# adria0/plonk-by-fingers

Measured on AMD Instinct MI355X. Metric: NTT elements/sec (Goldilocks, n=2^20 per GPU, natural order, bit-exact vs src/fft.rs), higher is better.
Workload: dtype u64 (Goldilocks p=2^64-2^32+1); 1 GPU; Goldilocks forward NTT, batch 32 x 2^20; n_per_gpu=1048576, n_global=1048576, batch=32, passes=default (2^20: 10,10)

## Files before the change

plonk-by-fingers_amd/csrc/ntt_gl.hpp:

```cpp
#pragma once
#include "ntt_kernels.hpp"

#ifdef PBF_GL_NOMATH
#define PBF_GL_MATH(x) do { } while (0)
#else
#define PBF_GL_MATH(x) x
#endif
#ifdef PBF_GL_NOMEM
#define PBF_GL_NOMEM_ON 1
#else
#define PBF_GL_NOMEM_ON 0
#endif

namespace pbf {

struct GlPassArgs {
  const uint64_t* in;
  uint64_t* out;
  const uint64_t* twpass;
  const uint64_t* tw0;
  const uint64_t* tw1;
  const uint64_t* tc;
  const uint64_t* tws_a;
  const uint64_t* tws_b;
  uint64_t n;
  uint32_t log_n;
  uint32_t log_ns;
  uint32_t tw_bits;
  uint32_t blocks_per_poly;
  uint32_t batch;
  uint32_t scaled;
  uint32_t out_split_log;
  uint32_t xcd_kmajor;
  uint64_t in_pitch, out_pitch;
  const uint64_t* post_tw;
  uint32_t skip_pass_tw;
  const uint64_t* cs_tab;
  const uint64_t* cs_tab1;
  uint32_t cs_bits;
  uint64_t cs_len;
};

template <int K>
__device__ __forceinline__ uint64_t gl_pow2(uint64_t x) {
  constexpr int RAW = ((K % 192) + 192) % 192;
  if constexpr (RAW == 0) {
    return x;
  } else if constexpr (RAW > 160) {
    return gl_div_pow2<192 - RAW>(x);
  } else {
    using T = ShiftKind<RAW>;
    const uint64_t y = apply_shift<Goldilocks, T>(x);
    if constexpr (T::NEG) {
      const FieldArgs f{};
      return Goldilocks::sub(0, y, f);
    } else {
      return y;
    }
  }
}

template <int E64, int Q1, int S2 = 1>
__device__ __forceinline__ void gl_stage_b_twiddle(uint64_t* v) {
  if constexpr (S2 < 16) {
    v[S2] = gl_pow2<(E64 * S2 * Q1) % 192>(v[S2]);
    gl_stage_b_twiddle<E64, Q1, S2 + 1>(v);
  }
}

template <int E64, int Q, int E = 1>
__device__ __forceinline__ void gl_post_twiddle_br(uint64_t* v) {
  if constexpr (E < 16) {
    v[bitrev_c(E, 4)] = gl_pow2<(E64 * E * Q) % 192>(v[bitrev_c(E, 4)]);
    gl_post_twiddle_br<E64, Q, E + 1>(v);
  }
}
template <int E64, int WV, int U = 0>
__device__ __forceinline__ void gl_rg3_c_shift(uint64_t* x) {
  if constexpr (U < 4) {
    constexpr int g = WV + 4 * U;
    x[U * 4 + 1] = gl_pow2<(E64 * g) % 192>(x[U * 4 + 1]);
    x[U * 4 + 2] = gl_pow2<(E64 * 2 * g) % 192>(x[U * 4 + 2]);
    x[U * 4 + 3] = gl_pow2<(E64 * 3 * g) % 192>(x[U * 4 + 3]);
    gl_rg3_c_shift<E64, WV, U + 1>(x);
  }
}

template <int LOGR, int TILE>
struct GlShape {
  static constexpr int R = 1 << LOGR;
  static constexpr int LOGC = LOGR - 6;
  static constexpr int C = 1 << LOGC;
  static constexpr int W = TILE / R;
  static constexpr int NT = TILE / 16;
  static constexpr int WPQ = NT / 256;
#ifdef PBF_GL_PAD_Y
  static constexpr bool YX = false;
#else
  static constexpr bool YX = W == 16 && C > 1;
#endif
  static constexpr int YP = (YX ? 64 : 65) * W;
  static constexpr int LDS = (C * YP > TILE) ? C * YP : TILE;
  static constexpr bool LDS32K = LDS * 8 <= 32768;
  static constexpr int NSUB_C = (64 * W) / NT;
  __host__ __device__ static constexpr int ysw(int k1) {
    return W <= 32 ? (k1 / (32 / W)) & (W - 1) : (k1 & 31);
  }
  __host__ __device__ static constexpr int yidx(int r2, int k1, int w) {
    return r2 * YP + (YX ? (k1 ^ (r2 & 1)) : k1) * W + (w ^ ysw(k1));
  }
};

__device__ __forceinline__ void gl_tile_coords(const GlPassArgs& a, uint32_t tile, uint32_t tiles, uint32_t* poly,
                                               uint32_t* kb) {
  if (a.xcd_kmajor == 1) {
    const uint32_t v = (tile & 7) * (tiles >> 3) + (tile >> 3);
    *kb = v / a.batch;
    *poly = v % a.batch;
  } else if (a.xcd_kmajor == 2) {
    const uint32_t v = (tile & 7) * (tiles >> 3) + (tile >> 3);
    *poly = v / a.blocks_per_poly;
    *kb = v % a.blocks_per_poly;
  } else {
    *poly = tile / a.blocks_per_poly;
    *kb = tile % a.blocks_per_poly;
  }
}

__device__ __forceinline__ uint64_t gl_cs_factor(const GlPassArgs& a, uint64_t i) {
  const FieldArgs f{};
  if (a.cs_tab1) return Goldilocks::mul(a.cs_tab[i & ((1ull << a.cs_bits) - 1)], a.cs_tab1[i >> a.cs_bits], f);
  return a.cs_tab[i];
}

constexpr int GL_STORES = 16;

template <int LOGR, int E64, bool FIRST, int TILE, int RG = 0, int CS = 0>
__device__ __forceinline__ void gl_tile(const GlPassArgs& a, uint64_t* lds, uint32_t tile, uint32_t tiles, int t) {
  using Sh = GlShape<LOGR, TILE>;
  constexpr int C = Sh::C, LOGC = Sh::LOGC, W = Sh::W, NT = Sh::NT, YP = Sh::YP;
  (void)YP;
  static_assert(Sh::NSUB_C * C == GL_STORES, "stores per thread");
  static_assert(RG == 0 || (LOGR == 8 && TILE == 4096 && FIRST == (RG == 1)), "RG shape");
  static_assert(CS == 0 || (FIRST == (CS == 1) && (RG == 0 || RG == 2 * CS - 1)), "CS 1: first pass, CS 2: last pass");
  const FieldArgs f{};
  using G = Goldilocks;
  uint32_t poly, kb;
  gl_tile_coords(a, tile, tiles, &poly, &kb);
  if constexpr (PBF_GL_NOMEM_ON) kb &= 1, poly = 0;
  const uint64_t j0 = (uint64_t)kb * W;
  const uint64_t* in = a.in + (uint64_t)poly * a.in_pitch;
  const uint64_t stride = a.n >> LOGR;

  uint64_t v[16];
  if constexpr (CS == 1) {
#pragma unroll
    for (int h = 0; h < 2; ++h) {
      uint64_t tw[8];
#pragma unroll
      for (int uu = 0; uu < 2; ++uu) {
        const int idx = t + NT * (2 * h + uu);
        const int w = idx % W, r2 = (idx / W) % C, s2 = idx / (C * W);
#pragma unroll
        for (int s1 = 0; s1 < 4; ++s1) {
          const uint64_t i = (j0 + w) + (uint64_t)(16 * C * s1 + C * s2 + r2) * stride;
          const bool on = i < a.cs_len;
          v[8 * h + uu * 4 + s1] = on ? in[i] : 0;
          tw[uu * 4 + s1] = on ? gl_cs_factor(a, i) : 0;
        }
      }
#pragma unroll
      for (int m = 0; m < 8; ++m) v[8 * h + m] = G::mul(v[8 * h + m], tw[m], f);
    }
  } else {
#pragma unroll
    for (int u = 0; u < 4; ++u) {
      const int idx = t + NT * u;
      const int w = idx % W, r2 = (idx / W) % C, s2 = idx / (C * W);
#pragma unroll
      for (int s1 = 0; s1 < 4; ++s1) {
        const int r = 16 * C * s1 + C * s2 + r2;
        v[u * 4 + s1] = in[(j0 + w) + (uint64_t)r * stride];
      }
    }
  }
  uint64_t t3[RG == 3 ? 2 : 1];
  if constexpr (RG == 3) {
    const int wave = t >> 6, q1 = wave / Sh::WPQ, rw = (wave % Sh::WPQ) * 64 + (t & 63);
    const int r2 = rw / W, w = rw % W;
    const uint64_t X = ((uint64_t)q1 << 16) + j0 + w;
    t3[0] = a.tws_a[((uint64_t)r2 << 18) + X];
    t3[1] = a.tws_b[X];
  }
  if constexpr (!FIRST && RG != 3) if (!a.skip_pass_tw) {
    const uint64_t kmask = (1ull << a.log_ns) - 1;
#pragma unroll
    for (int h = 0; h < 2; ++h) {
      uint64_t tw[8];
#pragma unroll
      for (int uu = 0; uu < 2; ++uu) {
        const int u = 2 * h + uu;
        const int idx = t + NT * u;
        const int w = idx % W, r2 = (idx / W) % C, s2 = idx / (C * W);
        const uint64_t k = (j0 + w) & kmask;
#pragma unroll
        for (int s1 = 0; s1 < 4; ++s1) {
          const uint64_t r = (uint64_t)(16 * C * s1 + C * s2 + r2);
          if (a.twpass) {
            tw[uu * 4 + s1] = a.twpass[(r << a.log_ns) + k];
          } else if (a.tws_a) {
            tw[uu * 4 + s1] = G::mul(a.tws_b[(uint64_t)kb * Sh::R + r], a.tws_a[r * W + w], f);
          } else {
            const uint64_t e = ((r * k) << (a.log_n - a.log_ns - LOGR)) & (a.n - 1);
            tw[uu * 4 + s1] = G::mul(a.tw0[e & ((1ull << a.tw_bits) - 1)], a.tw1[e >> a.tw_bits], f);
          }
        }
      }
#pragma unroll
      for (int m = 0; m < 8; ++m) PBF_GL_MATH(v[8 * h + m] = G::mul(v[8 * h + m], tw[m], f));
#ifdef PBF_GL_NOMATH
#pragma unroll
      for (int m = 0; m < 8; ++m) v[8 * h + m] ^= tw[m];
#endif
    }
  }
#pragma unroll
  for (int u = 0; u < 4; ++u) PBF_GL_MATH((dft_reg<G, 2, sub_root_exp(E64, 2)>(v + u * 4, nullptr, f)));
#pragma unroll
  for (int u = 0; u < 4; ++u) {
    const int idx = t + NT * u;
    const int s2 = idx / (C * W), rw = idx % (C * W);
#pragma unroll
    for (int q1 = 0; q1 < 4; ++q1) lds[(q1 * 16 + s2) * (C * W) + rw] = v[u * 4 + bitrev_c(q1, 2)];
  }
  __syncthreads();

  {
    const int wave = t >> 6;
    const int q1 = wave / Sh::WPQ;
    const int rw = (wave % Sh::WPQ) * 64 + (t & 63);
#pragma unroll
    for (int s2 = 0; s2 < 16; ++s2) v[s2] = lds[(q1 * 16 + s2) * (C * W) + rw];
#ifndef PBF_GL_NOMATH
    if constexpr (RG == 3) {
      uint64_t p = t3[0];
      const uint64_t d = t3[1];
#pragma unroll
      for (int s2 = 0; s2 < 16; ++s2) {
        v[s2] = G::mul(v[s2], p, f);
        if (s2 < 15) p = G::mul(p, d, f);
      }
    } else {
      switch (__builtin_amdgcn_readfirstlane(q1)) {
        case 1: gl_stage_b_twiddle<E64, 1>(v); break;
        case 2: gl_stage_b_twiddle<E64, 2>(v); break;
        case 3: gl_stage_b_twiddle<E64, 3>(v); break;
        default: break;
      }
    }
    dft_reg<G, 4, sub_root_exp(E64, 4)>(v, nullptr, f);
#endif
    __syncthreads();
    const int r2 = rw / W, w = rw % W;
#pragma unroll
    for (int q2 = 0; q2 < 16; ++q2) {
      const int k1 = q1 + 4 * q2;
      lds[Sh::yidx(r2, k1, w)] = v[bitrev_c(q2, 4)];
    }
  }
  __syncthreads();

  auto c_map = [&](int u, int* k1, int* w) {
    const int idx = t + NT * u;
    if constexpr (FIRST) {
      *k1 = idx & 63;
      *w = idx >> 6;
    } else {
      *k1 = idx / W;
      *w = idx % W;
    }
  };
  uint64_t x[Sh::NSUB_C * C];
#pragma unroll
  for (int u = 0; u < Sh::NSUB_C; ++u) {
    int k1, w;
    c_map(u, &k1, &w);
#pragma unroll
    for (int r2 = 0; r2 < C; ++r2) x[u * C + r2] = lds[Sh::yidx(r2, k1, w)];
  }
  if constexpr (RG == 3) {
    switch (__builtin_amdgcn_readfirstlane(t >> 6)) {
      case 0: gl_rg3_c_shift<E64, 0>(x); break;
      case 1: gl_rg3_c_shift<E64, 1>(x); break;
      case 2: gl_rg3_c_shift<E64, 2>(x); break;
      default: gl_rg3_c_shift<E64, 3>(x); break;
    }
  } else if constexpr (RG == 1) {
    const uint64_t* tc = a.tc + ((j0 >> 12) & 15) * 256;
#pragma unroll
    for (int u = 0; u < Sh::NSUB_C; ++u) {
      int k1, w;
      c_map(u, &k1, &w);
      uint64_t tw[C];
#pragma unroll
      for (int r2 = 0; r2 < C; ++r2) tw[r2] = tc[r2 * 64 + k1];
#pragma unroll
      for (int r2 = 0; r2 < C; ++r2) x[u * C + r2] = G::mul(x[u * C + r2], tw[r2], f);
    }
  } else {
    uint64_t tw[Sh::NSUB_C * C];
    const int r2lo = a.scaled ? 0 : 1;
#pragma unroll
    for (int u = 0; u < Sh::NSUB_C; ++u) {
      int k1, w;
      c_map(u, &k1, &w);
#pragma unroll
      for (int r2 = 0; r2 < C; ++r2) tw[u * C + r2] = (r2 >= r2lo) ? a.tc[r2 * 64 + k1] : 1;
    }
    if (a.scaled) {
#pragma unroll
      for (int m = 0; m < Sh::NSUB_C * C; ++m) PBF_GL_MATH(x[m] = G::mul(x[m], tw[m], f));
    } else {
#pragma unroll
      for (int u = 0; u < Sh::NSUB_C; ++u)
#pragma unroll
        for (int r2 = 1; r2 < C; ++r2) {
          PBF_GL_MATH(x[u * C + r2] = G::mul(x[u * C + r2], tw[u * C + r2], f));
#ifdef PBF_GL_NOMATH
          x[u * C + r2] ^= tw[u * C + r2];
#endif
        }
    }
  }
  if constexpr (C > 1) {
#pragma unroll
    for (int u = 0; u < Sh::NSUB_C; ++u) PBF_GL_MATH((dft_reg<G, LOGC, sub_root_exp(E64, LOGC)>(x + u * C, nullptr, f)));
  }

  if constexpr (FIRST) {
    uint64_t* o = a.out + (uint64_t)poly * a.out_pitch;
#pragma unroll
    for (int u = 0; u < Sh::NSUB_C; ++u) {
      int k1, w;
      c_map(u, &k1, &w);
      const uint64_t base = (j0 + w) << LOGR;
      if (a.post_tw) {
        uint64_t tw[C];
#pragma unroll
        for (int k2 = 0; k2 < C; ++k2) tw[k2] = a.post_tw[base + k1 + 64 * k2];
#pragma unroll
        for (int k2 = 0; k2 < C; ++k2) x[u * C + bitrev_c(k2, LOGC)] = G::mul(x[u * C + bitrev_c(k2, LOGC)], tw[k2], f);
      }
#pragma unroll
      for (int k2 = 0; k2 < C; ++k2)
        if (!PBF_GL_NOMEM_ON || x[u * C + bitrev_c(k2, LOGC)] == 0x123456789ull)
          o[base + k1 + 64 * k2] = x[u * C + bitrev_c(k2, LOGC)];
    }
  } else {
    const uint64_t ns_mask = (1ull << a.log_ns) - 1;
    uint64_t* out = a.out + (uint64_t)poly * a.out_pitch;
    const uint32_t sl = a.out_split_log;
#pragma unroll
    for (int u = 0; u < Sh::NSUB_C; ++u) {
      int k1, w;
      c_map(u, &k1, &w);
      const uint64_t j = j0 + w;
      const uint64_t base = ((j >> a.log_ns) << (a.log_ns + LOGR)) + (j & ns_mask);
      if (sl == 0) {
        if constexpr (CS == 2) {
          uint64_t tw[C];
#pragma unroll
          for (int k2 = 0; k2 < C; ++k2) tw[k2] = gl_cs_factor(a, base + ((uint64_t)(k1 + 64 * k2) << a.log_ns));
#pragma unroll
          for (int k2 = 0; k2 < C; ++k2) x[u * C + bitrev_c(k2, LOGC)] = G::mul(x[u * C + bitrev_c(k2, LOGC)], tw[k2], f);
        }
#pragma unroll
        for (int k2 = 0; k2 < C; ++k2)
          if (!PBF_GL_NOMEM_ON || x[u * C + bitrev_c(k2, LOGC)] == 0x123456789ull)
            out[base + ((uint64_t)(k1 + 64 * k2) << a.log_ns)] = x[u * C + bitrev_c(k2, LOGC)];
      } else {
        const uint64_t smask = (1ull << sl) - 1;
#pragma unroll
        for (int k2 = 0; k2 < C; ++k2) {
          const uint64_t kk = base + ((uint64_t)(k1 + 64 * k2) << a.log_ns);
          a.out[((((kk >> sl) * a.batch) + poly) << sl) + (kk & smask)] = x[u * C + bitrev_c(k2, LOGC)];
        }
      }
    }
  }
}

template <int LOGR, int TILE>
__device__ __forceinline__ void gl_shape_checks() {
  using Sh = GlShape<LOGR, TILE>;
  static_assert(LOGR >= 6 && LOGR <= 10, "radix 2^6 .. 2^10");
  static_assert(Sh::LDS * 8 <= (TILE > 8192 ? 160 : 80) * 1024, "LDS budget");
  static_assert(Sh::W >= 8 && Sh::WPQ >= 1, "tile shape");
}

template <int LOGR, int E64, bool FIRST, int TILE, int RG = 0, int CS = 0>
__global__ void __launch_bounds__(TILE / 16)
__attribute__((amdgpu_waves_per_eu((FIRST || RG) && GlShape<LOGR, TILE>::LDS32K ? 5 : 4)))
ntt_gl_pass_kernel(GlPassArgs a) {
  gl_shape_checks<LOGR, TILE>();
  __shared__ __attribute__((aligned(16))) uint64_t lds[GlShape<LOGR, TILE>::LDS];
  const uint32_t tiles = a.blocks_per_poly * a.batch;
  gl_tile<LOGR, E64, FIRST, TILE, RG, CS>(a, lds, blockIdx.x, tiles, threadIdx.x);
}

template <int E64>
__global__ void __launch_bounds__(256) __attribute__((amdgpu_waves_per_eu(4))) ntt_gl_rg2_kernel(GlPassArgs a) {
  constexpr int W = 16;
  __shared__ __attribute__((aligned(16))) uint64_t lds[16 * 16 * W];
  const FieldArgs f{};
  using G = Goldilocks;
  const uint32_t tiles = a.blocks_per_poly * a.batch;
  uint32_t poly, kb;
  gl_tile_coords(a, blockIdx.x, tiles, &poly, &kb);
  const int t = threadIdx.x, w = t % W, a1h = t / W;
  const uint64_t j0 = (uint64_t)kb * W, j = j0 + w;
  const uint32_t c = (uint32_t)(j0 >> 6) & 3, a1l = (uint32_t)(j0 >> 14) & 3;
  const uint64_t* in = a.in + (uint64_t)poly * a.in_pitch;
  const uint64_t stride = a.n >> 8;
  uint64_t v[16], tw[16];
#pragma unroll
  for (int a2l = 0; a2l < 16; ++a2l) v[a2l] = in[j + (uint64_t)(a2l * 16 + a1h) * stride];
  const uint64_t* t2 = a.twpass + ((uint64_t)(a1l + 4 * a1h) << 12) + (j & 255);
#pragma unroll
  for (int d = 0; d < 16; ++d) tw[d] = t2[256 * d];
  switch (__builtin_amdgcn_readfirstlane(c)) {
    case 1: gl_stage_b_twiddle<E64, 1>(v); break;
    case 2: gl_stage_b_twiddle<E64, 2>(v); break;
    case 3: gl_stage_b_twiddle<E64, 3>(v); break;
    default: break;
  }
  dft_reg<G, 4, sub_root_exp(E64, 4)>(v, nullptr, f);
#pragma unroll
  for (int d = 0; d < 16; ++d) lds[d * 256 + (a1h ^ (d & 3)) * W + w] = G::mul(v[bitrev_c(d, 4)], tw[d], f);
  __syncthreads();
  const int d2 = t / W;
#pragma unroll
  for (int h = 0; h < 16; ++h) v[h] = lds[d2 * 256 + (h ^ (d2 & 3)) * W + w];
  dft_reg<G, 4, sub_root_exp(E64, 4)>(v, nullptr, f);
  switch (__builtin_amdgcn_readfirstlane(a1l)) {
    case 1: gl_post_twiddle_br<E64, 1>(v); break;
    case 2: gl_post_twiddle_br<E64, 2>(v); break;
    case 3: gl_post_twiddle_br<E64, 3>(v); break;
    default: break;
  }
  uint64_t* out = a.out + (uint64_t)poly * a.out_pitch;
  const uint64_t base = ((j >> 8) << 16) + (j & 255);
#pragma unroll
  for (int e = 0; e < 16; ++e) out[base + ((uint64_t)(d2 + 16 * e) << 8)] = v[bitrev_c(e, 4)];
}

}
```

plonk-by-fingers_amd/csrc/ntt_kernels.hpp:

```cpp
#pragma once
#include "field.hpp"

namespace pbf {

#ifdef PBF_NTT_TIMING_MODES
#define PBF_DBG(a, bit) (((a).dbg & (bit)) != 0)
#else
#define PBF_DBG(a, bit) false
#endif

struct PassArgs {
  const uint64_t* in;
  uint64_t* out;
  const uint64_t* tw0;
  const uint64_t* tw1;
  const uint64_t* rtab;
  const uint64_t* twfull;
  const uint64_t* twpass;
  uint64_t n;
  uint64_t n_inv;
  uint32_t log_n;
  uint32_t log_ns;
  uint32_t tw_bits;
  uint32_t blocks_per_poly;
// ... 5 lines not shown
  uint32_t xcd_kmajor;
  FieldArgs f;
};

__host__ __device__ constexpr int ntt_nstages(int logr, int lq) { return (logr + lq - 1) / lq; }
__host__ __device__ constexpr int ntt_stage_logq(int logr, int s, int lq) {
  return (logr % lq == 0) ? lq : (s == 0 ? logr % lq : lq);
}
__host__ __device__ constexpr int ntt_stage_logl(int logr, int s, int lq) {
  int l = 0;
  for (int i = 0; i < s; ++i) l += ntt_stage_logq(logr, i, lq);
  return l;
}
__host__ __device__ constexpr int bitrev_c(int x, int bits) {
  int r = 0;
  for (int i = 0; i < bits; ++i) r |= ((x >> i) & 1) << (bits - 1 - i);
  return r;
}

template <class F>
__device__ __forceinline__ uint64_t tw_pow(const PassArgs& a, uint64_t e) {
  uint64_t lo = a.tw0[e & ((1ull << a.tw_bits) - 1)];
  uint64_t hi = a.tw1[e >> a.tw_bits];
  return F::mul(lo, hi, a.f);
}

template <int RAW_>
struct ShiftKind {
  static constexpr int RAW = ((RAW_ % 192) + 192) % 192;
  static constexpr bool NEG0 = RAW >= 96;
  static constexpr int S0 = NEG0 ? RAW - 96 : RAW;
  static constexpr bool DIV = S0 > 64;
  static constexpr bool NEG = DIV ? !NEG0 : NEG0;
  static constexpr int S = DIV ? 96 - S0 : S0;
};
template <int E, int LOGQ, int H, int A>
struct TwShift : ShiftKind<(E * A * ((1 << LOGQ) / (2 * H))) % 192> {};

template <class F, class T>
__device__ __forceinline__ uint64_t apply_shift(uint64_t d) {
  if constexpr (T::DIV) return gl_div_pow2<T::S>(d);
  else return F::template mul_pow2<T::S>(d);
}

template <class F, int LOGQ, int E, int H, int A>
__device__ __forceinline__ void dif_bfly(uint64_t* v, int blk, const uint64_t* wq, const FieldArgs& f) {
  constexpr int Q = 1 << LOGQ;
  const uint64_t x = v[blk + A], y = v[blk + A + H];
  v[blk + A] = F::add(x, y, f);
  if constexpr (A == 0) {
    v[blk + A + H] = F::sub(x, y, f);
  } else if constexpr (E < 0) {
    v[blk + A + H] = F::mul(F::sub(x, y, f), wq[A * (Q / (2 * H))], f);
  } else {
    using T = TwShift<E, LOGQ, H, A>;
    const uint64_t d = T::NEG ? F::sub(y, x, f) : F::sub(x, y, f);
    v[blk + A + H] = apply_shift<F, T>(d);
  }
}

template <class F, int LOGQ, int E, int H, int A>
__device__ __forceinline__ void dif_row(uint64_t* v, const uint64_t* wq, const FieldArgs& f) {
  if constexpr (A < H) {
    constexpr int Q = 1 << LOGQ;
#pragma unroll
    for (int blk = 0; blk < Q; blk += 2 * H) dif_bfly<F, LOGQ, E, H, A>(v, blk, wq, f);
    dif_row<F, LOGQ, E, H, A + 1>(v, wq, f);
  }
}

template <class F, int LOGQ, int E, int H>
__device__ __forceinline__ void dif_levels(uint64_t* v, const uint64_t* wq, const FieldArgs& f) {
  if constexpr (H >= 1) {
    dif_row<F, LOGQ, E, H, 0>(v, wq, f);
    dif_levels<F, LOGQ, E, H / 2>(v, wq, f);
  }
}

template <class F, int LOGQ, int E>
__device__ __forceinline__ void dft_reg(uint64_t* v, const uint64_t* wq, const FieldArgs& f) {
  dif_levels<F, LOGQ, E, (1 << LOGQ) / 2>(v, wq, f);
}

__host__ __device__ constexpr int sub_root_exp(int e64, int logq) {
  return e64 < 0 ? -1 : (e64 * (64 >> logq)) % 192;
}

template <bool DB>
__device__ __forceinline__ void tile_barrier() {
  if constexpr (DB) {
    asm volatile("s_waitcnt lgkmcnt(0)" ::: "memory");
    __builtin_amdgcn_s_barrier();
  } else {
    __syncthreads();
  }
}

template <int LOGR, int W, int NT, int LQ>
__device__ __forceinline__ void tile_load(uint64_t* v, const PassArgs& a, const uint64_t* in, uint64_t j0, int t) {
  constexpr int R = 1 << LOGR;
  constexpr int PER = (R * W) / NT;
  constexpr int Q = 1 << ntt_stage_logq(LOGR, 0, LQ);
#pragma unroll
  for (int u = 0; u < PER / Q; ++u) {
    const int sub = t + NT * u;
    const int w = sub % W, i = sub / W;
#pragma unroll
    for (int c = 0; c < Q; ++c) {
      const int r = i + c * (R / Q);
      v[u * Q + c] = PBF_DBG(a, 1) ? (uint64_t)(t * 0x9E3779B9u + r) * 0x100000001ull
                                 : in[(j0 + w) + (uint64_t)r * (a.n >> LOGR)];
    }
  }
}

template <class F, int LOGR, int W, int NT, int LQ, int E64, int S>
__device__ __forceinline__ void ntt_stage(uint64_t* v, uint64_t* buf, const uint64_t* rt, const uint64_t* wq,
                                          const PassArgs& a, uint64_t* out, uint64_t j0, int t) {
  constexpr int R = 1 << LOGR;
  constexpr int PER = (R * W) / NT;
  constexpr int NST = ntt_nstages(LOGR, LQ);
  constexpr int LOGQ = ntt_stage_logq(LOGR, S, LQ);
  constexpr int Q = 1 << LOGQ;
  constexpr int L = 1 << ntt_stage_logl(LOGR, S, LQ);
  constexpr int NSUB = PER / Q;
  constexpr bool LAST = (S == NST - 1);
  const uint64_t n = a.n;
  if constexpr (S == 0) {
    if (a.log_ns > 0) {
      const uint64_t kmask = (1ull << a.log_ns) - 1;
      if (a.twpass) {
        uint64_t tw[PER];
#pragma unroll
        for (int u = 0; u < NSUB; ++u) {
          const int sub = t + NT * u;
          const int w = sub % W, i = sub / W;
          const uint64_t k = (j0 + w) & kmask;
#pragma unroll
          for (int c = 0; c < Q; ++c) tw[u * Q + c] = a.twpass[((uint64_t)(i + c * (R / Q)) << a.log_ns) + k];
        }
#pragma unroll
        for (int m = 0; m < PER; ++m) v[m] = F::mul(v[m], tw[m], a.f);
      } else {
#pragma unroll
        for (int u = 0; u < NSUB; ++u) {
          const int sub = t + NT * u;
          const int w = sub % W, i = sub / W;
          const uint64_t k = (j0 + w) & kmask;
#pragma unroll
          for (int c = 0; c < Q; ++c) {
            const uint64_t r = i + c * (R / Q);
            const uint64_t e = ((r * k) << (a.log_n - a.log_ns - LOGR)) & (n - 1);
            if (e) v[u * Q + c] = F::mul(v[u * Q + c], tw_pow<F>(a, e), a.f);
          }
        }
      }
    }
  } else {
#pragma unroll
    for (int u = 0; u < NSUB; ++u) {
      const int sub = t + NT * u;
      const int w = sub % W, i = sub / W;
      const int k = i % L;
#pragma unroll
      for (int c = 0; c < Q; ++c) {
        const uint64_t x = buf[(i + c * (R / Q)) * W + w];
// ... 261 lines not shown
```

plonk-by-fingers_amd/csrc/ntt_launch.hip:

```cpp
#include <cstdlib>
#include <cstring>
#include <mutex>
#include "internal.hpp"
#include "ntt_gl.hpp"

namespace pbf {

bool hinv(uint64_t a, uint64_t m, uint64_t* out) {
  __int128 s = 0, old_s = 1, r = m, old_r = a % m;
  while (r != 0) {
    __int128 q = old_r / r, t;
    t = old_r - q * r; old_r = r; r = t;
    t = old_s - q * s; old_s = s; s = t;
  }
  if (old_r != 1) return false;
  if (old_s < 0) old_s += m;
  *out = (uint64_t)old_s;
  return true;
}

bool field_for(uint64_t m, FieldKind* kind, FieldArgs* fa) {
  fa->m = m;
  fa->mu = 0;
  if (m == GOLDILOCKS) { *kind = FIELD_GOLDILOCKS; return true; }
// ... 257 lines not shown
                     G);
  PBF_HIP(hipGetLastError());
  return 0;
}

int make_two_level(uint64_t m, uint64_t root, uint64_t n, TwoLevel* t) {
  uint32_t log_n = 0;
  while ((1ull << log_n) < n) ++log_n;
  t->bits = (log_n + 1) / 2;
  t->root = root;
  std::vector<uint64_t> t0(1ull << t->bits), t1((n >> t->bits) ? (n >> t->bits) : 1);
  uint64_t x = 1 % m;
  for (size_t i = 0; i < t0.size(); ++i) { t0[i] = x; x = hmul(x, root, m); }
  uint64_t step = x, y = 1 % m;
  for (size_t i = 0; i < t1.size(); ++i) { t1[i] = y; y = hmul(y, step, m); }
  int rc = upload(t->t0, t0);
  return rc ? rc : upload(t->t1, t1);
}

template <class F>
static int combine_typed(const FieldArgs& fa, const TwoLevel& tl, uint32_t G, uint64_t rank, const uint64_t* in,
                         uint64_t* out, uint64_t nl, uint32_t batch, int inverse, hipStream_t s) {
  CombineArgs a;
  a.recv = in; a.out = out;
  a.tw0 = (const uint64_t*)tl.t0.p; a.tw1 = (const uint64_t*)tl.t1.p; a.tw_bits = tl.bits;
  a.nl = nl; a.s = nl / G; a.rank = rank; a.n_mask = (uint64_t)G * nl - 1; a.batch = batch; a.f = fa;
  a.scale = 1;
  if (inverse) {
    uint64_t ginv;
    if (!hinv(G % fa.m, fa.m, &ginv)) return fail(2, "G has no inverse");
    a.scale = ginv;
  }
  for (int i = 0; i < 8; ++i) a.wg[i] = 0;
  const uint64_t wG = hpow(tl.root, nl, fa.m);
  uint64_t x = 1 % fa.m;
  for (uint32_t i = 0; i < G; ++i) { a.wg[i] = x; x = hmul(x, wG, fa.m); }
  const uint64_t total = (nl / G) * batch;
  void (*fn)(CombineArgs) = nullptr;
  switch (G) {
    case 2: fn = inverse ? shard_split_inv_kernel<F, 2> : shard_combine_kernel<F, 2>; break;
    case 4: fn = inverse ? shard_split_inv_kernel<F, 4> : shard_combine_kernel<F, 4>; break;
    case 8: fn = inverse ? shard_split_inv_kernel<F, 8> : shard_combine_kernel<F, 8>; break;
    default: return fail(1, "world size must be 2, 4 or 8");
  }
  hipLaunchKernelGGL(fn, dim3(grid_for(total)), dim3(256), 0, s, a);
  PBF_HIP(hipGetLastError());
  return 0;
}

int launch_shard_combine(FieldKind k, const FieldArgs& fa, const TwoLevel& tl, uint32_t G, uint64_t rank,
                         const uint64_t* in, uint64_t* out, uint64_t nl, uint32_t batch, int inverse, hipStream_t s) {
  if (k == FIELD_GOLDILOCKS) return combine_typed<Goldilocks>(fa, tl, G, rank, in, out, nl, batch, inverse, s);
  return combine_typed<Mod32>(fa, tl, G, rank, in, out, nl, batch, inverse, s);
}

typedef void (*GlPassFn)(GlPassArgs);

static int gl_tile(int logr) { return logr >= 10 ? 8192 : 4096; }

template <int E>
static GlPassFn gl_fn_e(int logr, bool first) {
  switch (logr) {
    case 6: return first ? ntt_gl_pass_kernel<6, E, true, 4096> : ntt_gl_pass_kernel<6, E, false, 4096>;
    case 7: return first ? ntt_gl_pass_kernel<7, E, true, 4096> : ntt_gl_pass_kernel<7, E, false, 4096>;
    case 8: return first ? ntt_gl_pass_kernel<8, E, true, 4096> : ntt_gl_pass_kernel<8, E, false, 4096>;
    case 9: return first ? ntt_gl_pass_kernel<9, E, true, 4096> : ntt_gl_pass_kernel<9, E, false, 4096>;
    case 10: return first ? ntt_gl_pass_kernel<10, E, true, 8192> : ntt_gl_pass_kernel<10, E, false, 8192>;
    default: return nullptr;
  }
}

template <int E>
static GlPassFn gl_fn_cs(int logr, int cs) {
  switch (logr) {
    case 6: return cs == 1 ? ntt_gl_pass_kernel<6, E, true, 4096, 0, 1> : ntt_gl_pass_kernel<6, E, false, 4096, 0, 2>;
    case 7: return cs == 1 ? ntt_gl_pass_kernel<7, E, true, 4096, 0, 1> : ntt_gl_pass_kernel<7, E, false, 4096, 0, 2>;
    case 8: return cs == 1 ? ntt_gl_pass_kernel<8, E, true, 4096, 0, 1> : ntt_gl_pass_kernel<8, E, false, 4096, 0, 2>;
    case 9: return cs == 1 ? ntt_gl_pass_kernel<9, E, true, 4096, 0, 1> : ntt_gl_pass_kernel<9, E, false, 4096, 0, 2>;
    case 10: return cs == 1 ? ntt_gl_pass_kernel<10, E, true, 8192, 0, 1> : ntt_gl_pass_kernel<10, E, false, 8192, 0, 2>;
    default: return nullptr;
  }
}

template <int E>
static GlPassFn gl_fn_rg(int pass) {
  if (pass == 0) return ntt_gl_pass_kernel<8, E, true, 4096, 1>;
  if (pass == 1) return ntt_gl_rg2_kernel<E>;
  return ntt_gl_pass_kernel<8, E, false, 4096, 3>;
}
template <int E>
static GlPassFn gl_fn_rg_cs(int cs) {
  return cs == 1 ? ntt_gl_pass_kernel<8, E, true, 4096, 1, 1> : ntt_gl_pass_kernel<8, E, false, 4096, 3, 2>;
}

static int run_gl_group(const NttPlan& p, const uint64_t* d_in, uint64_t* d_out, size_t batch, DevBuf& s0,
                        DevBuf& s1, hipStream_t stream, uint32_t split_log, size_t soff = 0,
                        const GlCoset* cs = nullptr);

int ForkSet::ensure(int streams) {
  if (streams > GL_MAX_STREAMS) streams = GL_MAX_STREAMS;
  if (streams > 1 && !fork) PBF_HIP(hipEventCreateWithFlags(&fork, hipEventDisableTiming));
  for (int i = 1; i < streams; ++i) {
    if (!aux[i]) PBF_HIP(hipStreamCreateWithFlags(&aux[i], hipStreamNonBlocking));
    if (!join[i]) PBF_HIP(hipEventCreateWithFlags(&join[i], hipEventDisableTiming));
  }
  return 0;
}

ForkSet::~ForkSet() {
  (void)hipSetDevice(device);
  for (int i = 1; i < GL_MAX_STREAMS; ++i) {
    if (aux[i]) {
      (void)hipStreamSynchronize(aux[i]);
      (void)hipStreamDestroy(aux[i]);
    }
    if (join[i]) (void)hipEventDestroy(join[i]);
  }
  if (fork) (void)hipEventDestroy(fork);
}

static int run_gl_passes(const NttPlan& p, const uint64_t* d_in, uint64_t* d_out, size_t batch, DevBuf& s0,
                         DevBuf& s1, hipStream_t stream, uint32_t split_log, ForkSet* fork, const GlCoset* cs) {
  const long long go = p.opts.num("ntt.group", -1);
  const size_t G = go >= 0 ? (size_t)go : (batch >= 8 ? 4 : batch);
  if (split_log != 0 || G == 0 || G >= batch)
    return run_gl_group(p, d_in, d_out, batch, s0, s1, stream, split_log, 0, cs);
  const size_t in_pitch = (cs && !p.inverse) ? cs->in_len : p.n;
  int ns = (int)p.opts.num("ntt.streams", 2);
  ns = ns < 1 ? 1 : (ns > GL_MAX_STREAMS ? GL_MAX_STREAMS : ns);
  if (!fork) ns = 1;
  hipStream_t sts[GL_MAX_STREAMS];
  sts[0] = stream;
  if (ns > 1) {
    int rc = fork->ensure(ns);
    if (rc) return rc;
    for (int i = 1; i < ns; ++i) sts[i] = fork->aux[i];
    PBF_HIP(hipEventRecord(fork->fork, stream));
    for (int i = 1; i < ns; ++i) PBF_HIP(hipStreamWaitEvent(sts[i], fork->fork, 0));
  }
  int gi = 0;
  for (size_t g0 = 0; g0 < batch; g0 += G, ++gi) {
    const size_t b = batch - g0 < G ? batch - g0 : G;
    const int rc = run_gl_group(p, d_in + g0 * in_pitch, d_out + g0 * p.n, b, s0, s1, sts[gi % ns], 0,
                                ns > 1 ? g0 * p.n : 0, cs);
    if (rc) return rc;
  }
  for (int i = 1; i < ns; ++i) {
    PBF_HIP(hipEventRecord(fork->join[i], sts[i]));
    PBF_HIP(hipStreamWaitEvent(stream, fork->join[i], 0));
  }
  return 0;
}

static int ensure_rg_tables(const NttPlan& p) {
  if (p.rg_built) return 0;
  const uint64_t m = p.m, n = p.n;
  const int inverse = p.inverse;
  uint64_t w = p.omega;
  if (inverse && !hinv(p.omega, m, &w)) return fail(1, "omega not invertible");
  int rc;
  const uint64_t w4096 = hpow(w, n / 4096, m);
  std::vector<uint64_t> tc1(4096);
  for (uint64_t a2l = 0; a2l < 16; ++a2l)
    for (uint64_t r2 = 0; r2 < 4; ++r2)
      for (uint64_t k1 = 0; k1 < 64; ++k1)
        tc1[a2l * 256 + r2 * 64 + k1] = hpow(w4096, ((a2l + 16 * r2) * k1) % 4096, m);
  std::vector<uint64_t> t2(1ull << 18);
  for (uint64_t a1 = 0; a1 < 64; ++a1) {
    const uint64_t st = hpow(w, 64 * a1, m);
    uint64_t y = 1;
    for (uint64_t K = 0; K < 4096; ++K) { t2[(a1 << 12) + K] = y; y = hmul(y, st, m); }
  }
  const uint64_t scale = inverse ? p.n_inv : 1;
  std::vector<uint64_t> tgc(4ull << 18), tgb(1ull << 18);
  {
    const uint64_t w4 = hpow(w, 4, m);
    uint64_t x1 = 1, x4 = 1;
    for (uint64_t X = 0; X < (1ull << 18); ++X) {
      tgb[X] = x4;
      uint64_t c = scale;
      for (uint64_t r2 = 0; r2 < 4; ++r2) {
        tgc[(r2 << 18) + X] = c;
        c = hmul(c, x1, m);
      }
      x1 = hmul(x1, w, m);
      x4 = hmul(x4, w4, m);
    }
  }
  if ((rc = upload(p.rg_tc1, tc1)) || (rc = upload(p.rg_t2, t2)) || (rc = upload(p.rg_tgc, tgc)) ||
      (rc = upload(p.rg_tgb, tgb)))
    return rc;
  p.rg_built = true;
  return 0;
}

static int run_gl_group(const NttPlan& p, const uint64_t* d_in, uint64_t* d_out, size_t batch, DevBuf& s0,
                        DevBuf& s1, hipStream_t stream, uint32_t split_log, size_t soff, const GlCoset* cs) {
  const size_t P = p.logr.size();
  const bool rg = p.rg && P == 3 && split_log == 0;
  if (cs && (split_log != 0 || P < 2)) return fail(1, "coset transform: unsupported plan");
  if (rg) {
    const int rc = ensure_rg_tables(p);
    if (rc) return rc;
  }
  uint32_t log_ns = 0;
  for (size_t i = 0; i < P; ++i) {
    const int lr = p.logr[i];
    const int tile = gl_tile(lr);
    GlPassFn fn = p.e64 == 39 ? gl_fn_e<39>(lr, log_ns == 0) : gl_fn_e<153>(lr, log_ns == 0);
    if (rg) fn = p.e64 == 39 ? gl_fn_rg<39>((int)i) : gl_fn_rg<153>((int)i);
    const int csv = !cs ? 0 : (!p.inverse && i == 0) ? 1 : (p.inverse && i == P - 1) ? 2 : 0;
    if (csv && rg) fn = p.e64 == 39 ? gl_fn_rg_cs<39>(csv) : gl_fn_rg_cs<153>(csv);
    else if (csv) fn = p.e64 == 39 ? gl_fn_cs<39>(lr, csv) : gl_fn_cs<153>(lr, csv);
    if (!fn) return fail(1, "no Goldilocks pass kernel for this radix");
    const uint64_t W = (uint64_t)tile >> lr;
    if ((p.n >> lr) % W) return fail(1, "transform too small for the pass tile");
    GlPassArgs a;
    a.in = (i == 0) ? d_in : (const uint64_t*)(((i - 1) & 1) ? s1.p : s0.p) + soff;
    a.out = (i == P - 1) ? d_out : (uint64_t*)((i & 1) ? s1.p : s0.p) + soff;
    a.in_pitch = a.out_pitch = p.n;
    a.twpass = (const uint64_t*)p.twpass[i]->p;
    a.tw0 = (const uint64_t*)p.tw0.p;
    a.tw1 = (const uint64_t*)p.tw1.p;
    a.tc = (const uint64_t*)p.tc[i]->p;
    const bool tws = !a.twpass && i == P - 1 && p.tws_a && (uint64_t)p.tws_w == W;
    a.tws_a = tws ? (const uint64_t*)p.tws_a->p : nullptr;
    a.tws_b = tws ? (const uint64_t*)p.tws_b->p : nullptr;
    a.n = p.n;
    a.log_n = p.log_n;
    a.log_ns = log_ns;
    a.tw_bits = p.tw_bits;
    a.blocks_per_poly = (uint32_t)((p.n >> lr) / W);
    a.batch = (uint32_t)batch;
    a.scaled = (p.inverse && i == P - 1) ? 1 : 0;
    a.out_split_log = (i == P - 1) ? split_log : 0;
    const uint64_t tiles = (uint64_t)a.blocks_per_poly * batch;
    if (tiles > 0x7fffffffull) return fail(1, "batch too large");
    a.xcd_kmajor = (log_ns > 0 && batch > 1 && tiles % 8 == 0) ? 1 : 0;
    a.post_tw = nullptr;
    a.skip_pass_tw = 0;
    if (P == 2 && split_log == 0 && p.twpass[1]->p) {
      if (i == 0) a.post_tw = (const uint64_t*)p.twpass[1]->p;
      else a.skip_pass_tw = 1;
    }
    if (a.post_tw && batch > 1 && tiles % 8 == 0) a.xcd_kmajor = 1;
    a.cs_tab = a.cs_tab1 = nullptr;
    a.cs_bits = 0;
    a.cs_len = 0;
    if (csv) {
      a.cs_tab = (const uint64_t*)cs->tabs->t0.p;
      a.cs_tab1 = (const uint64_t*)cs->tabs->t1.p;
      a.cs_bits = cs->tabs->bits;
      if (csv == 1) {
        a.cs_len = cs->in_len;
        a.in_pitch = cs->in_len;
      } else if (!rg) {
        a.tc = (const uint64_t*)cs->tabs->tc_last.p;
        a.scaled = 0;
      }
    }
    if (rg) {
      if (i == 0) a.tc = (const uint64_t*)p.rg_tc1.p;
      if (i == 1) a.twpass = (const uint64_t*)p.rg_t2.p;
      if (i == 2) {
        a.twpass = nullptr;
        a.tws_a = (const uint64_t*)p.rg_tgc.p;
        a.tws_b = (const uint64_t*)p.rg_tgb.p;
      }
      if (tiles % 8 == 0) a.xcd_kmajor = 2;
    }
    hipLaunchKernelGGL(fn, dim3((uint32_t)tiles), dim3(tile / 16), 0, stream, a);
    PBF_HIP(hipGetLastError());
    log_ns += lr;
  }
  return 0;
}

static int run_plan_impl(const NttPlan& p, const uint64_t* d_in, uint64_t* d_out, size_t batch, DevBuf& s0,
                         DevBuf& s1, hipStream_t stream, uint32_t split_log, ForkSet* fork, const GlCoset* cs) {
  if (batch == 0) return 0;
  if (p.n == 1) {
    if (d_in != d_out) PBF_HIP(hipMemcpyAsync(d_out, d_in, batch * 8, hipMemcpyDeviceToDevice, stream));
    return 0;
  }
  if (p.logr.empty()) {
    if (p.kind == FIELD_GOLDILOCKS)
      hipLaunchKernelGGL(ntt_small_kernel<Goldilocks>, dim3(batch), dim3(256), 0, stream, d_in, d_out,
                         (const uint64_t*)p.small_tw.p, p.log_n, p.n_inv, (uint32_t)p.inverse, p.fa);
    else
      hipLaunchKernelGGL(ntt_small_kernel<Mod32>, dim3(batch), dim3(256), 0, stream, d_in, d_out,
                         (const uint64_t*)p.small_tw.p, p.log_n, p.n_inv, (uint32_t)p.inverse, p.fa);
    PBF_HIP(hipGetLastError());
    return 0;
  }
  const size_t P = p.logr.size();
  const size_t bytes = batch * p.n * 8;
  int rc = s0.ensure(bytes);
  if (!rc && P > 2) rc = s1.ensure(bytes);
  if (rc) return rc;
  uint32_t log_ns = 0;
  if (p.gl) return run_gl_passes(p, d_in, d_out, batch, s0, s1, stream, split_log, fork, cs);
  if (cs) return fail(1, "coset transform: not a Goldilocks standard-root plan");
  for (size_t i = 0; i < P; ++i) {
    const int lr = p.logr[i];
    PassCfg cfg = pass_cfg(lr);
    PassFn fn = pass_fn(p.kind, p.e64, lr, cfg);
    for (int w : {16, 8, 4}) {
      if (fn) break;
      cfg = PassCfg{w, 4};
      fn = pass_fn(p.kind, p.e64, lr, cfg);
    }
    if (!fn) return fail(1, "no kernel for this radix");
    const int W = cfg.w;
    PassArgs a;
    a.in = (i == 0) ? d_in : (const uint64_t*)(((i - 1) & 1) ? s1.p : s0.p);
    a.out = (i == P - 1) ? d_out : (uint64_t*)((i & 1) ? s1.p : s0.p);
    a.tw0 = (const uint64_t*)p.tw0.p;
    a.tw1 = (const uint64_t*)p.tw1.p;
    a.rtab = (const uint64_t*)p.rtab[i]->p;
    a.twfull = nullptr;
    a.twpass = (const uint64_t*)p.twpass[i]->p;
    a.n = p.n;
    a.n_inv = p.n_inv;
    a.log_n = p.log_n;
    a.log_ns = log_ns;
    a.tw_bits = p.tw_bits;
    a.blocks_per_poly = (uint32_t)((p.n >> lr) / W);
    a.scale = (p.inverse && i == P - 1) ? 1 : 0;
    a.out_split_log = (i == P - 1) ? split_log : 0;
    a.dbg = 0;
    a.batch = (uint32_t)batch;
    a.f = p.fa;
    const int nt = (W << lr) >> cfg.lq;
    const uint64_t blocks = (uint64_t)a.blocks_per_poly * batch;
    if (blocks > 0x7fffffffull) return fail(1, "batch too large");
    const uint32_t grid = (uint32_t)blocks;
    a.xcd_kmajor = (log_ns > 0 && batch > 1 && grid % 8 == 0) ? 1 : 0;
    hipLaunchKernelGGL(fn, dim3(grid), dim3(nt), 0, stream, a);
    PBF_HIP(hipGetLastError());
    log_ns += lr;
  }
  return 0;
}

static uint32_t log2_ceil(uint64_t x) {
  uint32_t l = 0;
  while ((1ull << l) < x) ++l;
  return l;
}

static int coset_tabs(const NttPlan& p, uint64_t shift, uint64_t len, const CosetTabs** out) {
  const uint64_t m = p.m;
  CosetTabs* t = nullptr;
  for (auto& c : p.coset)
    if (c->shift == shift) t = c.get();
  if (t && t->len >= len) {
    t->stamp = ++p.coset_clock;
    *out = t;
    return 0;
  }
  if (!t) {
    if (p.coset.size() >= COSET_SHIFTS_PER_PLAN) {
      size_t old = 0;
      for (size_t i = 1; i < p.coset.size(); ++i)
        if (p.coset[i]->stamp < p.coset[old]->stamp) old = i;
      p.coset.erase(p.coset.begin() + old);
    }
    p.coset.emplace_back(new CosetTabs());
    t = p.coset.back().get();
    t->shift = shift;
  } else {
    PBF_HIP(hipDeviceSynchronize());
  }
  t->len = 0;
  uint64_t s = shift, c = 1 % m;
  if (p.inverse) {
    if (!hinv(shift, m, &s)) return fail(1, "shift has no inverse");
    if (p.gl && !p.rg) c = p.n_inv;
  }
// ... 195 lines not shown
```

Measured before the change: 103.8 billion elements/s.

## Fold twiddle negations into DIF butterflies and specialize second Goldilocks pass

Stage-B power-of-two twiddles now apply only the shift magnitude, and their signs travel as a compile-time mask through the first radix-2 levels of the register DFT. Each butterfly absorbs the sign by swapping add/sub operands, which removes the separate negation subtractions. A specialized second-pass kernel (SP) for plain two-pass 2^10 x 2^10 forward plans turns log_ns, split and scaled handling into compile-time constants and drops the runtime pass-twiddle branch. Scratch buffers are also sized to group*streams polynomials instead of the whole batch, with per-stream offsets, which cuts scratch memory footprint and may improve cache locality.

```diff
diff --git a/plonk-by-fingers_amd/csrc/ntt_gl.hpp b/plonk-by-fingers_amd/csrc/ntt_gl.hpp
--- a/plonk-by-fingers_amd/csrc/ntt_gl.hpp
+++ b/plonk-by-fingers_amd/csrc/ntt_gl.hpp
@@ -41,8 +41,12 @@
   uint64_t cs_len;
 };
 
+__host__ __device__ constexpr bool gl_pow2_neg(int k) {
+  const int raw = ((k % 192) + 192) % 192;
+  return raw > 64 && raw <= 160;
+}
 template <int K>
-__device__ __forceinline__ uint64_t gl_pow2(uint64_t x) {
+__device__ __forceinline__ uint64_t gl_pow2_abs(uint64_t x) {
   constexpr int RAW = ((K % 192) + 192) % 192;
   if constexpr (RAW == 0) {
     return x;
@@ -50,13 +54,18 @@
     return gl_div_pow2<192 - RAW>(x);
   } else {
     using T = ShiftKind<RAW>;
-    const uint64_t y = apply_shift<Goldilocks, T>(x);
-    if constexpr (T::NEG) {
-      const FieldArgs f{};
-      return Goldilocks::sub(0, y, f);
-    } else {
-      return y;
-    }
+    static_assert(T::NEG == gl_pow2_neg(K), "sign of 2^K");
+    return apply_shift<Goldilocks, T>(x);
+  }
+}
+template <int K>
+__device__ __forceinline__ uint64_t gl_pow2(uint64_t x) {
+  const uint64_t y = gl_pow2_abs<K>(x);
+  if constexpr (gl_pow2_neg(K)) {
+    const FieldArgs f{};
+    return Goldilocks::sub(0, y, f);
+  } else {
+    return y;
   }
 }
 
@@ -66,6 +75,25 @@
     v[S2] = gl_pow2<(E64 * S2 * Q1) % 192>(v[S2]);
     gl_stage_b_twiddle<E64, Q1, S2 + 1>(v);
   }
+}
+template <int E64, int Q1, int S2 = 1>
+__device__ __forceinline__ void gl_stage_b_twiddle_abs(uint64_t* v) {
+  if constexpr (S2 < 16) {
+    v[S2] = gl_pow2_abs<(E64 * S2 * Q1) % 192>(v[S2]);
+    gl_stage_b_twiddle_abs<E64, Q1, S2 + 1>(v);
+  }
+}
+__host__ __device__ constexpr unsigned gl_stage_b_negmask(int e64, int q1) {
+  unsigned m = 0;
+  for (int s2 = 1; s2 < 16; ++s2) m |= gl_pow2_neg((e64 * s2 * q1) % 192) ? 1u << s2 : 0u;
+  return m;
+}
+constexpr int GL_B_LEVELS = 2;
+template <int E64, int Q1>
+__device__ __forceinline__ void gl_stage_b_head(uint64_t* v) {
+  const FieldArgs f{};
+  gl_stage_b_twiddle_abs<E64, Q1>(v);
+  dft_reg_signed<Goldilocks, 4, sub_root_exp(E64, 4), gl_stage_b_negmask(E64, Q1), GL_B_LEVELS>(v, f);
 }
 
 template <int E64, int Q, int E = 1>
@@ -135,12 +163,13 @@
 
 constexpr int GL_STORES = 16;
 
-template <int LOGR, int E64, bool FIRST, int TILE, int RG = 0, int CS = 0>
+template <int LOGR, int E64, bool FIRST, int TILE, int RG = 0, int CS = 0, int SP = 0>
 __device__ __forceinline__ void gl_tile(const GlPassArgs& a, uint64_t* lds, uint32_t tile, uint32_t tiles, int t) {
   using Sh = GlShape<LOGR, TILE>;
   constexpr int C = Sh::C, LOGC = Sh::LOGC, W = Sh::W, NT = Sh::NT, YP = Sh::YP;
   (void)YP;
   static_assert(Sh::NSUB_C * C == GL_STORES, "stores per thread");
+  static_assert(SP == 0 || (!FIRST && RG == 0 && CS == 0 && SP <= 2), "SP: second pass of a plain two-pass plan");
   static_assert(RG == 0 || (LOGR == 8 && TILE == 4096 && FIRST == (RG == 1)), "RG shape");
   static_assert(CS == 0 || (FIRST == (CS == 1) && (RG == 0 || RG == 2 * CS - 1)), "CS 1: first pass, CS 2: last pass");
   const FieldArgs f{};
@@ -192,7 +221,7 @@
     t3[0] = a.tws_a[((uint64_t)r2 << 18) + X];
     t3[1] = a.tws_b[X];
   }
-  if constexpr (!FIRST && RG != 3) if (!a.skip_pass_tw) {
+  if constexpr (!FIRST && RG != 3 && SP == 0) if (!a.skip_pass_tw) {
     const uint64_t kmask = (1ull << a.log_ns) - 1;
 #pragma unroll
     for (int h = 0; h < 2; ++h) {
@@ -250,15 +279,16 @@
         v[s2] = G::mul(v[s2], p, f);
         if (s2 < 15) p = G::mul(p, d, f);
       }
+      dft_reg<G, 4, sub_root_exp(E64, 4)>(v, nullptr, f);
     } else {
       switch (__builtin_amdgcn_readfirstlane(q1)) {
-        case 1: gl_stage_b_twiddle<E64, 1>(v); break;
-        case 2: gl_stage_b_twiddle<E64, 2>(v); break;
-        case 3: gl_stage_b_twiddle<E64, 3>(v); break;
-        default: break;
-      }
-    }
-    dft_reg<G, 4, sub_root_exp(E64, 4)>(v, nullptr, f);
+        case 1: gl_stage_b_head<E64, 1>(v); break;
+        case 2: gl_stage_b_head<E64, 2>(v); break;
+        case 3: gl_stage_b_head<E64, 3>(v); break;
+        default: gl_stage_b_head<E64, 0>(v); break;
+      }
+      dft_reg_tail<G, 4, sub_root_exp(E64, 4), GL_B_LEVELS>(v, f);
+    }
 #endif
     __syncthreads();
     const int r2 = rw / W, w = rw % W;
@@ -309,7 +339,8 @@
     }
   } else {
     uint64_t tw[Sh::NSUB_C * C];
-    const int r2lo = a.scaled ? 0 : 1;
+    const bool scaled = SP == 0 && a.scaled;
+    const int r2lo = scaled ? 0 : 1;
 #pragma unroll
     for (int u = 0; u < Sh::NSUB_C; ++u) {
       int k1, w;
@@ -317,7 +348,7 @@
 #pragma unroll
       for (int r2 = 0; r2 < C; ++r2) tw[u * C + r2] = (r2 >= r2lo) ? a.tc[r2 * 64 + k1] : 1;
     }
-    if (a.scaled) {
+    if (scaled) {
 #pragma unroll
       for (int m = 0; m < Sh::NSUB_C * C; ++m) PBF_GL_MATH(x[m] = G::mul(x[m], tw[m], f));
     } else {
@@ -357,32 +388,33 @@
           o[base + k1 + 64 * k2] = x[u * C + bitrev_c(k2, LOGC)];
     }
   } else {
-    const uint64_t ns_mask = (1ull << a.log_ns) - 1;
+    const uint32_t lns = SP == 2 ? (uint32_t)LOGR : a.log_ns;
+    const uint64_t ns_mask = (1ull << lns) - 1;
     uint64_t* out = a.out + (uint64_t)poly * a.out_pitch;
-    const uint32_t sl = a.out_split_log;
+    const uint32_t sl = SP != 0 ? 0u : a.out_split_log;
 #pragma unroll
     for (int u = 0; u < Sh::NSUB_C; ++u) {
       int k1, w;
       c_map(u, &k1, &w);
       const uint64_t j = j0 + w;
-      const uint64_t base = ((j >> a.log_ns) << (a.log_ns + LOGR)) + (j & ns_mask);
+      const uint64_t base = ((j >> lns) << (lns + LOGR)) + (j & ns_mask);
       if (sl == 0) {
         if constexpr (CS == 2) {
           uint64_t tw[C];
 #pragma unroll
-          for (int k2 = 0; k2 < C; ++k2) tw[k2] = gl_cs_factor(a, base + ((uint64_t)(k1 + 64 * k2) << a.log_ns));
+          for (int k2 = 0; k2 < C; ++k2) tw[k2] = gl_cs_factor(a, base + ((uint64_t)(k1 + 64 * k2) << lns));
 #pragma unroll
           for (int k2 = 0; k2 < C; ++k2) x[u * C + bitrev_c(k2, LOGC)] = G::mul(x[u * C + bitrev_c(k2, LOGC)], tw[k2], f);
         }
 #pragma unroll
         for (int k2 = 0; k2 < C; ++k2)
           if (!PBF_GL_NOMEM_ON || x[u * C + bitrev_c(k2, LOGC)] == 0x123456789ull)
-            out[base + ((uint64_t)(k1 + 64 * k2) << a.log_ns)] = x[u * C + bitrev_c(k2, LOGC)];
+            out[base + ((uint64_t)(k1 + 64 * k2) << lns)] = x[u * C + bitrev_c(k2, LOGC)];
       } else {
         const uint64_t smask = (1ull << sl) - 1;
 #pragma unroll
         for (int k2 = 0; k2 < C; ++k2) {
-          const uint64_t kk = base + ((uint64_t)(k1 + 64 * k2) << a.log_ns);
+          const uint64_t kk = base + ((uint64_t)(k1 + 64 * k2) << lns);
           a.out[((((kk >> sl) * a.batch) + poly) << sl) + (kk & smask)] = x[u * C + bitrev_c(k2, LOGC)];
         }
       }
@@ -398,14 +430,14 @@
   static_assert(Sh::W >= 8 && Sh::WPQ >= 1, "tile shape");
 }
 
-template <int LOGR, int E64, bool FIRST, int TILE, int RG = 0, int CS = 0>
+template <int LOGR, int E64, bool FIRST, int TILE, int RG = 0, int CS = 0, int SP = 0>
 __global__ void __launch_bounds__(TILE / 16)
 __attribute__((amdgpu_waves_per_eu((FIRST || RG) && GlShape<LOGR, TILE>::LDS32K ? 5 : 4)))
 ntt_gl_pass_kernel(GlPassArgs a) {
   gl_shape_checks<LOGR, TILE>();
   __shared__ __attribute__((aligned(16))) uint64_t lds[GlShape<LOGR, TILE>::LDS];
   const uint32_t tiles = a.blocks_per_poly * a.batch;
-  gl_tile<LOGR, E64, FIRST, TILE, RG, CS>(a, lds, blockIdx.x, tiles, threadIdx.x);
+  gl_tile<LOGR, E64, FIRST, TILE, RG, CS, SP>(a, lds, blockIdx.x, tiles, threadIdx.x);
 }
 
 template <int E64>
diff --git a/plonk-by-fingers_amd/csrc/ntt_kernels.hpp b/plonk-by-fingers_amd/csrc/ntt_kernels.hpp
--- a/plonk-by-fingers_amd/csrc/ntt_kernels.hpp
+++ b/plonk-by-fingers_amd/csrc/ntt_kernels.hpp
@@ -111,6 +111,63 @@
   dif_levels<F, LOGQ, E, (1 << LOGQ) / 2>(v, wq, f);
 }
 
+__host__ __device__ constexpr bool dif_tw_neg(int e, int logq, int h, int a) {
+  const int raw = (e * a * ((1 << logq) / (2 * h))) % 192;
+  const bool neg0 = raw >= 96;
+  return (neg0 ? raw - 96 : raw) > 64 ? !neg0 : neg0;
+}
+template <int LOGQ, int E, int H>
+__host__ __device__ constexpr unsigned dif_level_mask(unsigned m) {
+  unsigned r = 0;
+  for (int i = 0; i < (1 << LOGQ) / 2; ++i) {
+    const int a = i % H, lo = (i / H) * 2 * H + a, hi = lo + H;
+    const bool nx = (m >> lo) & 1, ny = (m >> hi) & 1;
+    if (nx == ny) r |= nx ? 1u << lo : 0u;
+    else if (nx != dif_tw_neg(E, LOGQ, H, a)) r |= 1u << hi;
+  }
+  return r;
+}
+template <class F, int LOGQ, int E, int H, unsigned M, int I = 0>
+__device__ __forceinline__ void dif_level_s(uint64_t* v, const FieldArgs& f) {
+  if constexpr (I < (1 << LOGQ) / 2) {
+    constexpr int A = I % H, lo = (I / H) * 2 * H + A, hi = lo + H;
+    constexpr bool nx = (M >> lo) & 1, ny = (M >> hi) & 1;
+    using T = TwShift<E, LOGQ, H, A>;
+    static_assert(T::NEG == dif_tw_neg(E, LOGQ, H, A), "twiddle sign");
+    const uint64_t x = v[lo], y = v[hi];
+    uint64_t d;
+    if constexpr (nx == ny) {
+      v[lo] = F::add(x, y, f);
+      d = (nx != T::NEG) ? F::sub(y, x, f) : F::sub(x, y, f);
+    } else {
+      v[lo] = nx ? F::sub(y, x, f) : F::sub(x, y, f);
+      d = F::add(x, y, f);
+    }
+    v[hi] = apply_shift<F, T>(d);
+    dif_level_s<F, LOGQ, E, H, M, I + 1>(v, f);
+  }
+}
+template <class F, int LOGQ, int E, int H, int HSTOP, unsigned M>
+__device__ __forceinline__ void dif_levels_s(uint64_t* v, const FieldArgs& f) {
+  if constexpr (H > HSTOP) {
+    dif_level_s<F, LOGQ, E, H, M>(v, f);
+    dif_levels_s<F, LOGQ, E, H / 2, HSTOP, dif_level_mask<LOGQ, E, H>(M)>(v, f);
+  } else {
+#pragma unroll
+    for (int i = 0; i < (1 << LOGQ); ++i)
+      if ((M >> i) & 1) v[i] = F::sub(0, v[i], f);
+  }
+}
+template <class F, int LOGQ, int E, unsigned M, int LEVELS = LOGQ>
+__device__ __forceinline__ void dft_reg_signed(uint64_t* v, const FieldArgs& f) {
+  static_assert(E >= 0 && LOGQ <= 5 && LEVELS >= 1 && LEVELS <= LOGQ, "shift twiddles; one mask bit per element");
+  dif_levels_s<F, LOGQ, E, (1 << LOGQ) / 2, (((1 << LOGQ) / 2) >> LEVELS), M>(v, f);
+}
+template <class F, int LOGQ, int E, int LEVELS>
+__device__ __forceinline__ void dft_reg_tail(uint64_t* v, const FieldArgs& f) {
+  dif_levels<F, LOGQ, E, (((1 << LOGQ) / 2) >> LEVELS)>(v, nullptr, f);
+}
+
 __host__ __device__ constexpr int sub_root_exp(int e64, int logq) {
   return e64 < 0 ? -1 : (e64 * (64 >> logq)) % 192;
 }
diff --git a/plonk-by-fingers_amd/csrc/ntt_launch.hip b/plonk-by-fingers_amd/csrc/ntt_launch.hip
--- a/plonk-by-fingers_amd/csrc/ntt_launch.hip
+++ b/plonk-by-fingers_amd/csrc/ntt_launch.hip
@@ -363,6 +363,10 @@
   }
 }
 
+static GlPassFn gl_fn_sp10(bool same_radix) {
+  return same_radix ? ntt_gl_pass_kernel<10, 39, false, 8192, 0, 0, 2> : ntt_gl_pass_kernel<10, 39, false, 8192, 0, 0, 1>;
+}
+
 template <int E>
 static GlPassFn gl_fn_rg(int pass) {
   if (pass == 0) return ntt_gl_pass_kernel<8, E, true, 4096, 1>;
@@ -400,16 +404,29 @@
   if (fork) (void)hipEventDestroy(fork);
 }
 
+static void gl_schedule(const NttPlan& p, size_t batch, uint32_t split_log, const ForkSet* fork, size_t* G, int* ns) {
+  const long long go = p.opts.num("ntt.group", -1);
+  *G = go >= 0 ? (size_t)go : (batch >= 8 ? 4 : batch);
+  if (split_log != 0 || *G >= batch) *G = 0;
+  *ns = (int)p.opts.num("ntt.streams", 2);
+  *ns = *ns < 1 ? 1 : (*ns > GL_MAX_STREAMS ? GL_MAX_STREAMS : *ns);
+  if (!fork || *G == 0) *ns = 1;
+}
+
+static size_t gl_scratch_polys(const NttPlan& p, size_t batch, uint32_t split_log, const ForkSet* fork) {
+  size_t G;
+  int ns;
+  gl_schedule(p, batch, split_log, fork, &G, &ns);
+  return (G == 0 || G * ns > batch) ? batch : G * ns;
+}
+
 static int run_gl_passes(const NttPlan& p, const uint64_t* d_in, uint64_t* d_out, size_t batch, DevBuf& s0,
                          DevBuf& s1, hipStream_t stream, uint32_t split_log, ForkSet* fork, const GlCoset* cs) {
-  const long long go = p.opts.num("ntt.group", -1);
-  const size_t G = go >= 0 ? (size_t)go : (batch >= 8 ? 4 : batch);
-  if (split_log != 0 || G == 0 || G >= batch)
-    return run_gl_group(p, d_in, d_out, batch, s0, s1, stream, split_log, 0, cs);
+  size_t G;
+  int ns;
+  gl_schedule(p, batch, split_log, fork, &G, &ns);
+  if (G == 0) return run_gl_group(p, d_in, d_out, batch, s0, s1, stream, split_log, 0, cs);
   const size_t in_pitch = (cs && !p.inverse) ? cs->in_len : p.n;
-  int ns = (int)p.opts.num("ntt.streams", 2);
-  ns = ns < 1 ? 1 : (ns > GL_MAX_STREAMS ? GL_MAX_STREAMS : ns);
-  if (!fork) ns = 1;
   hipStream_t sts[GL_MAX_STREAMS];
   sts[0] = stream;
   if (ns > 1) {
@@ -423,7 +440,7 @@
   for (size_t g0 = 0; g0 < batch; g0 += G, ++gi) {
     const size_t b = batch - g0 < G ? batch - g0 : G;
     const int rc = run_gl_group(p, d_in + g0 * in_pitch, d_out + g0 * p.n, b, s0, s1, sts[gi % ns], 0,
-                                ns > 1 ? g0 * p.n : 0, cs);
+                                (size_t)(gi % ns) * G * p.n, cs);
     if (rc) return rc;
   }
   for (int i = 1; i < ns; ++i) {
@@ -493,6 +510,8 @@
     const int csv = !cs ? 0 : (!p.inverse && i == 0) ? 1 : (p.inverse && i == P - 1) ? 2 : 0;
     if (csv && rg) fn = p.e64 == 39 ? gl_fn_rg_cs<39>(csv) : gl_fn_rg_cs<153>(csv);
     else if (csv) fn = p.e64 == 39 ? gl_fn_cs<39>(lr, csv) : gl_fn_cs<153>(lr, csv);
+    const bool two_pass_tw = P == 2 && split_log == 0 && p.twpass[1]->p;
+    if (two_pass_tw && i == 1 && !cs && !p.inverse && p.e64 == 39 && lr == 10) fn = gl_fn_sp10(p.logr[0] == 10);
     if (!fn) return fail(1, "no Goldilocks pass kernel for this radix");
     const uint64_t W = (uint64_t)tile >> lr;
     if ((p.n >> lr) % W) return fail(1, "transform too small for the pass tile");
@@ -520,7 +539,7 @@
     a.xcd_kmajor = (log_ns > 0 && batch > 1 && tiles % 8 == 0) ? 1 : 0;
     a.post_tw = nullptr;
     a.skip_pass_tw = 0;
-    if (P == 2 && split_log == 0 && p.twpass[1]->p) {
+    if (two_pass_tw) {
       if (i == 0) a.post_tw = (const uint64_t*)p.twpass[1]->p;
       else a.skip_pass_tw = 1;
     }
@@ -575,7 +594,7 @@
     return 0;
   }
   const size_t P = p.logr.size();
-  const size_t bytes = batch * p.n * 8;
+  const size_t bytes = (p.gl ? gl_scratch_polys(p, batch, split_log, fork) : batch) * p.n * 8;
   int rc = s0.ensure(bytes);
   if (!rc && P > 2) rc = s1.ensure(bytes);
   if (rc) return rc;
```

Result: faster. 107.9 billion elements/s, median of 6 (+3.9%).
